# qianduoduolr/FGVC

Measured on AMD Instinct MI355X. Metric: frames/sec + ms/corr-volume, 480p 8-frame clip, 1/2/4/8 MI355X, higher is better.
Workload: dtype f16 + fp6 (e2m3) MFMA operands, f32 accumulate; top-k near-ties re-scored in f64 from f32 features

## Files before the change

### fgvc_amd/_lib.py

```python
from __future__ import annotations

import ctypes as C
import contextlib
import os

_HERE = os.path.dirname(os.path.abspath(__file__))
LIB_PATH = os.environ.get("FGVC_HIP_LIB") or os.path.join(_HERE, "lib", "libfgvc_hip.so")

FGVC_OK = 0
ERR_INVALID_ARG, ERR_UNSUPPORTED, ERR_LAUNCH = 1, 2, 3
NO_LIMIT = 0x3FFFFFFF
PAIR_MASKED = 1
WEIGHT_SOFTMAX, WEIGHT_COSINE, WEIGHT_RAW = 0, 1, 2

_p = C.c_void_p
_i = C.c_int
_f = C.c_float

SIGNATURES = {
    "fgvc_version": (C.c_char_p, []),
    "fgvc_last_error": (C.c_char_p, []),
    "fgvc_set_option": (_i, [C.c_char_p, _i]),
    "fgvc_r2max_for_radius": (_i, [_f]),
    "fgvc_normalize_chw_to_hwc_f32": (_i, [_p, _p, _i, _i, _i, _i, _i, _p]),
# ... 4 lines not shown
    "fgvc_split_f16f6p": (_i, [_p, _p, C.c_int64, _i, _p]),
    "fgvc_pair_topk_f16f6": (_i, [_p, _p, _p, _i, _i, _i, _i, _i, _i, _i, _i, _i, _i, _i, _p, _p, _p]),
    "fgvc_pair_topk_f16f6_runs": (_i, [_p, _p, _p, _i, _i, _i, _i, _i, _i, _i, _i, _i, _i, _i, _p, _i, _p, _p, _p]),
    "fgvc_split_f16f6x": (_i, [_p, _p, C.c_int64, _i, _p]),
    "fgvc_pair_topk_f16f6x": (_i, [_p, _p, _p, _i, _i, _i, _i, _i, _i, _i, _i, _i, _i, _i, _p, _p, _p]),
    "fgvc_pair_topk_f16f6x_runs": (_i, [_p, _p, _p, _i, _i, _i, _i, _i, _i, _i, _i, _i, _i, _i, _p, _i, _p, _p, _p]),
    "fgvc_merge_refine_workspace_bytes": (C.c_size_t, [_i, _i]),
    "fgvc_merge_refine_topk_f32": (_i, [_p, _p, _p, _p, _p, C.c_int64, _i, _p, C.c_int64, _i, _i, _i, _i, _i, _i, _i, _i, _i, _f, _i, _f, _i, _i, _i,
                                        _p, _p, _p, _p, _p]),
    "fgvc_pair_topk_f16x3_timed_out": (_i, []),
    "fgvc_pair_topk_f16x3_probe": (_i, [_p]),
    "fgvc_conv64_probe": (_i, [_p]),
    "fgvc_nchw_to_split_nhwc_f32": (_i, [_p, _p, _p, _i, _i, _i, _i, _i, _i, _p]),
    "fgvc_conv_split_f32": (_i, [_p, _p, _p, _p, _p, _p, _i, _i, _i, _i, _i, _i, _i, _i, _i, _p]),
    "fgvc_conv_split_fmt_f32": (_i, [_p, _p, _p, _p, _p, _p, _i, _i, _i, _i, _i, _i, _i, _i, _i, _i, _i, _i, _i, _p, _p]),
    "fgvc_conv_split_proj_fmt_f32": (_i, [_p, _p, _p, _p, _p, _p, _p, _p, _i, _i, _i, _i, _i, _i, _i, _i, _i, _i, _i, _i, _p, _p]),
    "fgvc_conv_split_bank_f16f6p_f32": (_i, [_p, _p, _p, _p, _p, _i, _i, _i, _i, _i, _i, _i, _i, _i, _i, _i, _p]),
    "fgvc_conv_split_bank_f16f6x_f32": (_i, [_p, _p, _p, _p, _p, _i, _i, _i, _i, _i, _i, _i, _i, _i, _i, _i, _p]),
    "fgvc_conv64_split_f32": (_i, [_p, _p, _p, _p, _p, _p, _i, _i, _i, _i, _i, _i, _p]),
    "fgvc_conv64_split_res_f32": (_i, [_p, _p, _p, _p, _p, _p, _p, _i, _i, _i, _i, _i, _i, _p]),
    "fgvc_conv64_split_fmt_f32": (_i, [_p, _p, _p, _p, _p, _p, _p, _i, _i, _i, _i, _i, _i, _i, _i, _i, _i, _p, _p]),
    "fgvc_conv_s2_split_f32": (_i, [_p, _p, _p, _p, _p, _i, _i, _i, _i, _i, _i, _i, _i, _i, _i, _i, _p]),
    "fgvc_conv_s2_split_fmt_f32": (_i, [_p, _p, _p, _p, _p, _i, _i, _i, _i, _i, _i, _i, _i, _i, _i, _i, _i, _i, _p, _p]),
    "fgvc_stem7_split_f32": (_i, [_p, _p, _p, _p, _p, _i, _i, _i, _i, _i, _i, _p]),
    "fgvc_stem7_split_fmt_f32": (_i, [_p, _p, _p, _p, _p, _i, _i, _i, _i, _i, _i, _i, _i, _p, _p]),
    "fgvc_nhwc_to_split_f32": (_i, [_p, _p, _i, _i, _i, _i, _i, _i, _i, _p]),
    "fgvc_normalize_nhwc_f32": (_i, [_p, _p, _i, _i, _i, _i, _i, _p]),
    "fgvc_normalize_split_nhwc_f32": (_i, [_p, _p, _p, _i, _i, _i, _i, _i, _p]),
    "fgvc_normalize_split_f16x2_nhwc_f32": (_i, [_p, _p, _p, _i, _i, _i, _i, _i, _p]),
    "fgvc_normalize_split_f16f6p_nhwc_f32": (_i, [_p, _p, _i, _i, _i, _i, _i, _p]),
    "fgvc_normalize_split_f16f6x_nhwc_f32": (_i, [_p, _p, _i, _i, _i, _i, _i, _p]),
    "fgvc_merge_topk_f32": (_i, [_p, _p, _p, _i, _i, _i, _i, _i, _f, _i, _p, _p, _p, _p]),
    "fgvc_propagate_topk_f32": (_i, [_p, _p, _i, _p, _p, _i, _i, _i, _i, _i, _i, _i, _p, _p]),
    "fgvc_corr_volume_f32": (_i, [_p, _p, _i, _i, _i, _f, _p, _p]),
    "fgvc_split_bf16": (_i, [_p, _p, C.c_int64, _i, _p]),
    "fgvc_corr_volume_bf16x3": (_i, [_p, _p, _i, _i, _i, _f, _p, _p]),
    "fgvc_corr_volume_bf16": (_i, [_p, _p, _i, _i, _i, _f, _p, _p]),
    "fgvc_split_f16f8": (_i, [_p, _p, C.c_int64, _i, _p]),
    "fgvc_corr_volume_f16f8": (_i, [_p, _p, _i, _i, _i, _f, _p, _p]),
    "fgvc_split_f16f6": (_i, [_p, _p, C.c_int64, _i, _p]),
    "fgvc_corr_volume_f16f6": (_i, [_p, _p, _i, _i, _i, _f, _p, _p]),
    "fgvc_debug_store_sweep_f32": (_i, [_p, C.c_int64, _i, _p]),
    "fgvc_dense_attend_splits": (_i, [_i, _i]),
    "fgvc_dense_attend_f32": (_i, [_p, _p, _i, _i, _i, _i, _i, _i, _i, _i, _i, _i, _i, _p, _i, _p]),
    "fgvc_dense_attend_finish_f32": (_i, [_p, _i, _i, _i, _i, _p, _p]),
    "fgvc_dense_kth_f32": (_i, [_p, _i, _i, _i, _p, _i, _p, _p]),
# ... 69 lines not shown
```

### fgvc_amd/csrc/capi.hip

```cpp
#include <stdarg.h>
#include <string.h>

#include "common.hpp"

namespace fgvc {

static thread_local char g_err[512] = "";

void set_error(const char* fmt, ...) {
  va_list ap;
  va_start(ap, fmt);
  vsnprintf(g_err, sizeof(g_err), fmt, ap);
  va_end(ap);
}

int pair_topk_launch(const float*, const float*, const int32_t*, int, int, int, int, int, int, int, int, int, int,
                     const uint8_t*, int32_t*, float*, hipStream_t);
int merge_topk_launch(const int32_t*, const float*, const int32_t*, int, int, int, int, int, float, int, int32_t*,
                      float*, float*, hipStream_t);
int normalize_launch(const float*, float*, int, int, int, int, int, hipStream_t);
int propagate_launch(const float*, const int32_t*, int, const int32_t*, const float*, int, int, int, int, int, int,
                     int, float*, hipStream_t);
int bn_act_launch(const float*, const float*, const float*, const float*, const float*, const float*, float, int, float*,
                  int, int, int, hipStream_t);
int gaussian_launch(const float*, int, int, int, int, float, float*, hipStream_t);
int softargmax_launch(const float*, int, int, int, int, int, int, const float*, float, double*, float*, hipStream_t);
int softargmax_bands();
int corr_volume_f32_launch(const float*, const float*, int, int, int, float, float*, hipStream_t);
int split_bf16_launch(const float*, uint16_t*, long long, int, hipStream_t);
int corr_volume_bf16_launch(const uint16_t*, const uint16_t*, int, int, int, float, float*, int, hipStream_t);
int local_merge_launch(const int32_t*, const float*, int, int, int, int, int, float, int32_t*, float*, float*,
                       hipStream_t);
int topk_coord_launch(const int32_t*, const float*, int, int, int, int, int, float*, hipStream_t);
int c2f_refine_launch(const int32_t*, const float*, const float*, const float*, int, int, int, int, int, int, int,
                      int, float, int, float*, int32_t*, float*, hipStream_t);

int conv_split_launch(const uint16_t*, const uint16_t*, const float*, const float*, uint16_t*, float*, int, int, int, int, int,
                      int, int, int, int, int, int, int, int, int*, hipStream_t, unsigned char* y_bank = nullptr, int bank_normalize = 1, const uint16_t* x2 = nullptr,
                      const uint16_t* w2 = nullptr, int Cin2 = 0, int bank_row_bytes = 1024);
int conv_s2_launch(const uint16_t*, const uint16_t*, const float*, uint16_t*, float*, int, int, int, int, int, int, int, int, int,
                   int, int, int, int, int*, hipStream_t);
int conv64_launch(const uint16_t*, const uint16_t*, const float*, const float*, const uint16_t*, uint16_t*, float*, int, int, int, int, int, int,
                  int, int, int, int, int*, hipStream_t);
int stem7_launch(const float*, const uint16_t*, const float*, uint16_t*, float*, int, int, int, int, int, int, int, int, int, int, int*,
                 hipStream_t);
int nchw_to_split_nhwc_launch(const float*, uint16_t*, float*, int, int, int, int, int, int, hipStream_t);
int normalize_nhwc_launch(const float*, float*, uint16_t*, int, int, int, int, int, int, hipStream_t);
int nhwc_to_split_launch(float*, uint16_t*, int, int, int, int, int, int, int, hipStream_t);

void set_conv_cot_cap(int);
void set_conv_narrow(int);
void set_conv64_variant(int);
int conv64_probe_read(long long*);
void set_conv_debug(int);
void set_corr6_skew(int);
void set_corr6_sdma(int);
void set_pair_debug(int);
void set_readout_prune(int);
void set_conv_s2_debug(int);
int split_f16x2_launch(const float*, uint16_t*, long long, int, hipStream_t);
int split_f16f6p_launch(const float*, unsigned char*, long long, int, hipStream_t);
int pair_topk_v7_launch(const uint16_t*, const uint16_t*, const int32_t*, int, int, int, int, int, int, int, int, int, const int32_t*, int,
                        int32_t*, float*, int, hipStream_t);
int pair_topk_v5_launch(const uint16_t*, const uint16_t*, const int32_t*, int, int, int, int, int, int, int, int, int, int, const int32_t*,
// ... 636 lines not shown

int fgvc_conv_s2_split_fmt_f32(const uint16_t* x, const uint16_t* w, const float* bias, uint16_t* y_split, float* y_f32, int N,
                               int H, int W, int Hp, int Wp, int Cin, int Cout, int KS, int Hop, int Wop, int relu, int out_fmt,
                               int out_scale_log2, int* overflow, void* stream) {
  FGVC_REQUIRE(x && w && bias && (y_split || y_f32), FGVC_ERR_INVALID_ARG, "fgvc_conv_s2_split_f32: null pointer");
  FGVC_REQUIRE(out_fmt >= 0 && out_fmt <= 3 && out_scale_log2 > -100 && out_scale_log2 < 100, FGVC_ERR_INVALID_ARG, "fgvc_conv_s2_split_fmt_f32: bad output format / scale");
  FGVC_REQUIRE(out_fmt == FGVC_ACT_BF16X2 || !y_split || overflow, FGVC_ERR_INVALID_ARG, "fgvc_conv_s2_split_fmt_f32: an f16-format output needs the overflow word");
  FGVC_REQUIRE(N >= 0 && H > 0 && W > 0, FGVC_ERR_INVALID_ARG, "fgvc_conv_s2_split_f32: bad shape");
  FGVC_REQUIRE(KS == 1 || KS == 3, FGVC_ERR_UNSUPPORTED, "fgvc_conv_s2_split_f32: kernel size %d (1 or 3, stride 2)", KS);
  FGVC_REQUIRE(Cin > 0 && Cin % 32 == 0 && Cout > 0 && Cout % 32 == 0, FGVC_ERR_UNSUPPORTED,
               "fgvc_conv_s2_split_f32: Cin=%d and Cout=%d must be multiples of 32", Cin, Cout);
  const int Ho = (H - 1) / 2 + 1, Wo = (W - 1) / 2 + 1;
  FGVC_REQUIRE(conv_pad_ok(H, W, Hp, Wp), FGVC_ERR_INVALID_ARG, "fgvc_conv_s2_split_f32: padded size %dx%d too small for %dx%d", Hp, Wp, H, W);
  FGVC_REQUIRE(!y_split || conv_pad_ok(Ho, Wo, Hop, Wop), FGVC_ERR_INVALID_ARG,
               "fgvc_conv_s2_split_f32: padded output size %dx%d too small for %dx%d", Hop, Wop, Ho, Wo);
  FGVC_REQUIRE(aligned16(x) && aligned16(w) && aligned16(bias) && aligned16(y_split) && aligned16(y_f32),
               FGVC_ERR_INVALID_ARG, "fgvc_conv_s2_split_f32: 16-byte alignment required");
  FGVC_REQUIRE((const void*)x != (const void*)y_split, FGVC_ERR_INVALID_ARG, "fgvc_conv_s2_split_f32: in-place not supported");
  if (N == 0) return FGVC_OK;
  return conv_s2_launch(x, w, bias, y_split, y_f32, N, Hp, Wp, Cin, Cout, KS, Ho, Wo, Hop, Wop, relu, out_fmt, out_scale_log2, overflow,
                        (hipStream_t)stream);
}

int fgvc_stem7_split_f32(const float* x, const uint16_t* w, const float* bias, uint16_t* y_split, float* y_f32, int N, int H,
                         int W, int Hop, int Wop, int relu, void* stream) {
  return fgvc_stem7_split_fmt_f32(x, w, bias, y_split, y_f32, N, H, W, Hop, Wop, relu, FGVC_ACT_BF16X2, 0, nullptr, stream);
}

int fgvc_stem7_split_fmt_f32(const float* x, const uint16_t* w, const float* bias, uint16_t* y_split, float* y_f32, int N, int H,
                             int W, int Hop, int Wop, int relu, int out_fmt, int out_scale_log2, int* overflow, void* stream) {
  FGVC_REQUIRE(x && w && bias && (y_split || y_f32), FGVC_ERR_INVALID_ARG, "fgvc_stem7_split_f32: null pointer");
  FGVC_REQUIRE(out_fmt == FGVC_ACT_BF16X2 || out_fmt == FGVC_ACT_F16F8, FGVC_ERR_UNSUPPORTED, "fgvc_stem7_split_fmt_f32: output format %d", out_fmt);
  FGVC_REQUIRE(out_fmt == FGVC_ACT_BF16X2 || !y_split || overflow, FGVC_ERR_INVALID_ARG,
               "fgvc_stem7_split_fmt_f32: an f16-format output needs the overflow word");
  FGVC_REQUIRE(out_scale_log2 > -100 && out_scale_log2 < 100, FGVC_ERR_INVALID_ARG, "fgvc_stem7_split_fmt_f32: scale exponent out of range");
  FGVC_REQUIRE(N >= 0 && H > 0 && W > 0, FGVC_ERR_INVALID_ARG, "fgvc_stem7_split_f32: bad shape");
  const int Ho = (H - 1) / 2 + 1, Wo = (W - 1) / 2 + 1;
  FGVC_REQUIRE(!y_split || conv_pad_ok(Ho, Wo, Hop, Wop), FGVC_ERR_INVALID_ARG,
               "fgvc_stem7_split_f32: padded output size %dx%d too small for %dx%d", Hop, Wop, Ho, Wo);
  FGVC_REQUIRE(aligned16(w) && aligned16(bias) && aligned16(y_split) && aligned16(y_f32) && ((uintptr_t)x & 3) == 0,
               FGVC_ERR_INVALID_ARG, "fgvc_stem7_split_f32: alignment (16 bytes; 4 for x)");
  if (N == 0) return FGVC_OK;
  return stem7_launch(x, w, bias, y_split, y_f32, N, H, W, Ho, Wo, Hop, Wop, relu, out_fmt, out_scale_log2, overflow, (hipStream_t)stream);
}

int fgvc_nhwc_to_split_f32(float* x, uint16_t* out, int N, int C, int H, int W, int Hp, int Wp, int relu, void* stream) {
// ... 72 lines not shown
```

### fgvc_amd/csrc/conv_s2.hip

```cpp
#include "common.hpp"

namespace fgvc {

struct ConvS2Params {
  const uint16_t* x;
  const uint16_t* w;
  const float* bias;
  uint16_t* y_split;
  float* y_f32;
  int N, Hp, Wp, Cin, Cout, Ho, Wo, Hop, Wop, relu;
  int n_ty, n_tx;
  int debug;
  float out_scale;
  int out_fmt;
  int* overflow;
};


__device__ __forceinline__ void s2_lds_dma_16(const void* src_lane, uint32_t lds_uniform) {
  asm volatile("s_mov_b32 m0, %1\n\ts_nop 0\n\tglobal_load_lds_dwordx4 %0, off" ::"v"(src_lane), "s"(lds_uniform) : "memory");
}
__device__ __forceinline__ uint32_t s2_lds_addr(const void* p) {
  return (uint32_t)(size_t)(const __attribute__((address_space(3))) unsigned char*)p;
}
__device__ __forceinline__ int s2_swz(int e, int s) { return e * 128 + ((s ^ ((e >> 1) & 7)) << 4); }

constexpr int S2_TR = 4;
constexpr int S2_NW = 2 * S2_TR;
constexpr int S2_CPG = 1;
constexpr int S2_RS = 144;

template <int KS>
__global__ __launch_bounds__(64 * S2_NW, 2) void conv_s2_kernel(ConvS2Params p) {
  constexpr int T = KS * KS;
  constexpr int NR = KS == 3 ? 2 * S2_TR + 1 : S2_TR;
  constexpr int NC = KS == 3 ? 65 : 32;
  constexpr int NE = NR * NC;
  constexpr int NG = (NE + 7) / 8;
// ... 180 lines not shown
    }
  }
}

static int g_conv_s2_debug = 0;
void set_conv_s2_debug(int v) { g_conv_s2_debug = v; }

int conv_s2_launch(const uint16_t* x, const uint16_t* w, const float* bias, uint16_t* y_split, float* y_f32, int N, int Hp,
                   int Wp, int Cin, int Cout, int KS, int Ho, int Wo, int Hop, int Wop, int relu, int out_fmt, int out_scale_log2,
                   int* overflow, hipStream_t s) {
  ConvS2Params p;
  p.out_fmt = out_fmt; p.out_scale = ldexpf(1.0f, out_scale_log2); p.overflow = overflow;
  p.x = x; p.w = w; p.bias = bias; p.y_split = y_split; p.y_f32 = y_f32;
  p.N = N; p.Hp = Hp; p.Wp = Wp; p.Cin = Cin; p.Cout = Cout; p.Ho = Ho; p.Wo = Wo; p.Hop = Hop; p.Wop = Wop; p.relu = relu;
  p.n_ty = cdiv(Ho, S2_TR); p.n_tx = cdiv(Wo, 32);
  p.debug = g_conv_s2_debug;
  dim3 grid(p.n_ty * p.n_tx * N, cdiv(Cout, 128));
  if (KS == 3) conv_s2_kernel<3><<<grid, 64 * S2_NW, 0, s>>>(p);
  else conv_s2_kernel<1><<<grid, 64 * S2_NW, 0, s>>>(p);
  FGVC_CHECK_LAUNCH("fgvc_conv_s2_split_f32");
  return FGVC_OK;
}

}
```

### fgvc_amd/mmpt_api/backbones.py

```python
from __future__ import annotations

import re
from typing import Sequence

import torch
import torch.nn as nn
import torch.nn.functional as F

from .registry import BACKBONES

_CAPTURING = [False]


class ConvBN(nn.Module):

    def __init__(self, cin, cout, k, stride=1, padding=0, dilation=1, relu=True):
        super().__init__()
        self.conv = nn.Conv2d(cin, cout, k, stride, padding, dilation, bias=False)
        self.bn = nn.BatchNorm2d(cout)
        self.relu = relu

    def forward(self, x, residual=None, relu=None):
        relu = self.relu if relu is None else relu
        y = self.conv(x)
# ... 80 lines not shown
            if self.torchvision_pretrain:
                load_torchvision_checkpoint(self, self.pretrained)
            elif isinstance(self.pretrained, str):
                load_checkpoint(self, self.pretrained)
            else:
                raise Exception("a state dict is only accepted as a torchvision checkpoint (resnet.py:590)")
            return
        for m in self.modules():
            if isinstance(m, nn.Conv2d):
                nn.init.kaiming_normal_(m.weight, mode="fan_out", nonlinearity="relu")
            elif isinstance(m, nn.BatchNorm2d):
                nn.init.constant_(m.weight, 1)
                nn.init.constant_(m.bias, 0)
        if self.zero_init_residual:
            for m in self.modules():
                if isinstance(m, BasicBlock):
                    nn.init.constant_(m.conv2.bn.weight, 0)
                elif isinstance(m, Bottleneck):
                    nn.init.constant_(m.conv3.bn.weight, 0)

    use_conv64 = True
    use_stem7 = True
    use_s2_conv = True
    conv64_f16f8 = True
    res_from_split = False
    use_split_conv = True
    arith = "f16f6"
    fold_projection = True
    layer1_whole_batch = True
    fuse_bank = True

    @staticmethod
    def supported_arith():
        return ("f16f6", "f16f8", "bf16x3", "f16x3")

    def set_arith(self, arith: str):
        if arith not in self.supported_arith():
            raise ValueError(f"arith={arith!r}: one of {self.supported_arith()}")
        if arith != self.arith:
            self.arith = arith
            self.reset_split_cache()

    def _generic_s1(self, cb) -> bool:
        c = cb.conv
        return c.stride == (1, 1) and not (self.use_conv64 and tuple(c.weight.shape) == (64, 64, 3, 3))

    def _is_conv64(self, cb) -> bool:
        c = cb.conv
        return bool(self.use_conv64 and c.stride == (1, 1) and tuple(c.weight.shape) == (64, 64, 3, 3))

    def _stem7_ok(self) -> bool:
        c1 = self.conv1.conv
        return bool(self.use_stem7 and c1.kernel_size == (7, 7) and c1.stride == (2, 2) and c1.padding == (3, 3) and c1.in_channels == 3
                    and c1.out_channels == 64 and c1.dilation == (1, 1) and self.conv1.relu)

    def _format_plan(self, last: int):
        from .. import ops
        fmt, bf = ops.ACT_FMT[self.arith], ops.ACT_BF16X2
        cache = self.__dict__.setdefault("_split_cache", {})
        key = ("fmt_plan", self.arith, last, self.use_conv64, self.use_s2_conv, self.use_stem7, self.conv64_f16f8)
        if key not in cache:
            blocks = [(s_i, b_i, blk) for s_i in range(last + 1) for b_i, blk in enumerate(getattr(self, self.res_layers[s_i]))]
            f64 = ops.ACT_F16F8 if (fmt in (ops.ACT_F16F8, ops.ACT_F16F6) and self.conv64_f16f8) else bf

            def reads(cb):
                if self._is_conv64(cb):
                    return f64
                return fmt if self._generic_s1(cb) else bf

            def can_write(cb, f):
                if f == bf:
                    return True
                if self._is_conv64(cb):
                    return f == ops.ACT_F16F8
                return self._generic_s1(cb) or (cb.conv.stride == (2, 2) and self.use_s2_conv)

            def wants(blk):
                f = reads(blk.conv1)
                return f if (blk.downsample is None or reads(blk.downsample) == f) else bf
            plan = {}
            f_in = wants(blocks[0][2]) if blocks else bf
            if f_in != bf and not (self._stem7_ok() and f_in == ops.ACT_F16F8):
                f_in = bf
# ... 241 lines not shown
            H, W = cur["H"], cur["W"]
            f_in, f_a, f_y = fmts[bi]
            s_in = cur.get("scale", 0)
            s_a = scales.get((si, bi, "a"), 0) if f_a != ACT_BF16X2 else 0
            s_y = scales.get((si, bi, "y"), 0) if f_y != ACT_BF16X2 else 0
            assert cur.get("fmt", ACT_BF16X2) == f_in, "split activation format mismatch between producer and consumer"

            def conv_s1(x_split, wb, in_fmt=ACT_BF16X2, in_scale=0, out_fmt=ACT_BF16X2, out_scale=0, **kw):
                if wb[3] == "conv64":
                    ops.conv64_split(x_split, wb[0], wb[1], H, W, in_fmt=in_fmt, in_scale_log2=in_scale + wb[2], out_fmt=out_fmt,
                                     out_scale_log2=out_scale, overflow=ovf, **kw)
                else:
                    ops.conv_split(x_split, wb[0], wb[1], H, W, in_fmt=in_fmt, in_scale_log2=in_scale + wb[2], out_fmt=out_fmt,
                                   out_scale_log2=out_scale, overflow=ovf, **kw)

            last_conv = bi == len(stage) - 1 and not cur["need_split"]
            proj = None
            x_in_split = cur["split"]
            if blk.conv1.conv.stride == (2, 2) and self.use_s2_conv:
                Hi, Wi = H, W
                H, W = (Hi - 1) // 2 + 1, (Wi - 1) // 2 + 1
                bufs = self._split_buffers((si, bi), N, Cout, H, W, dev, ("s_a", "s_y", "f_y", "f_idt"))
                buf = {k: v[lo:hi] for k, v in bufs.items()}
                ops.conv_s2_split(cur["split"], wt["ds"][0], wt["ds"][1], Hi, Wi, relu=False, out_f32=buf["f_idt"])
                idt = buf["f_idt"]
                ops.conv_s2_split(cur["split"], wt["c1"][0], wt["c1"][1], Hi, Wi, relu=True, out_split=buf["s_a"], out_fmt=f_a,
                                  out_scale_log2=s_a, overflow=ovf)
            elif blk.conv1.conv.stride != (1, 1):
                x_cl = cur["f32"].permute(0, 3, 1, 2)
                t1 = self._miopen_nhwc((si, bi, "c1"), blk.conv1, x_cl)
                idt = self._miopen_nhwc((si, bi, "ds"), blk.downsample, x_cl)
                _, H, W, _ = t1.shape
                bufs = self._split_buffers((si, bi), N, Cout, H, W, dev, ("s_a", "s_y", "f_y"))
                buf = {k: v[lo:hi] for k, v in bufs.items()}
                assert f_a == ACT_BF16X2
                ops.nhwc_to_split(t1, buf["s_a"], relu=True)
            else:
                bufs = self._split_buffers((si, bi), N, Cout, H, W, dev, ("s_a", "s_y", "f_y", "f_idt"))
                buf = {k: v[lo:hi] for k, v in bufs.items()}
                if blk.downsample is not None:
                    proj = self._projection_fold(blk, wt, si, bi, dev, f_in, f_a, s_in, s_a, Cout, last_conv and si == call["last"] and call.get("bank_of") is not None)
                if proj is not None:
                    idt = None
                elif blk.downsample is not None:
                    conv_s1(cur["split"], wt["ds"], f_in, s_in, relu=False, out_f32=buf["f_idt"])
                    idt = buf["f_idt"]
                elif self._identity_from_split(blk):
                    idt, idt_split = None, cur["split"]
                else:
                    idt = cur["f32"]
# ... 139 lines not shown
        for st in stages:
            x = st(x)
            outs.append(x)
        return outs[:-1], x, False, x.shape[-2], x.shape[-1]

    def forward(self, x, out_idx=None):
        want = tuple(out_idx) if out_idx is not None else self.out_indices
        last = max(want)
        earlier, y, nhwc, H, W = self._trunk(x, last, fresh=want)
        if nhwc:
            y = y.permute(0, 3, 1, 2)
        stage_out = earlier + [y]
        outs = [stage_out[i] for i in want]
        return outs[0] if len(outs) == 1 else tuple(outs)

    use_graph = "auto"
    graph_auto_max_px = 300_000

    def forward_hwc(self, x, normalize: bool = True, split_if=None, split_fmt: str = "bf16", out=None):
        want = self.use_graph is True or (self.use_graph == "auto" and x.dim() == 4 and x.shape[0] * x.shape[2] * x.shape[3] <= self.graph_auto_max_px)
        if not (want and x.is_cuda and not self.training and x.dtype == torch.float32) or torch.cuda.is_current_stream_capturing():
            return self.forward_hwc_eager(x, normalize, split_if, split_fmt, out)
        cache = self.__dict__.setdefault("_split_cache", {})
        sig = (self.arith, self.split_lanes, self.use_conv64, self.use_stem7, self.use_s2_conv, self.conv64_f16f8, self.res_from_split,
               self.use_split_conv, self.fuse_bank, self.fold_projection, self.layer1_whole_batch, tuple(self.out_indices))
        key = ("graph", tuple(x.shape), x.device, bool(normalize), split_fmt, split_if is not None, sig)
        ent = cache.get(key)
        if ent is None:
            cache[key] = "warm"
            return self.forward_hwc_eager(x, normalize, split_if, split_fmt, out)
        if ent == "warm":
            if self._scales(x.device) is None and self.arith != "bf16x3":
                return self.forward_hwc_eager(x, normalize, split_if, split_fmt, out)
            static_in = torch.empty_like(x)
            static_in.copy_(x)
            self.forward_hwc_eager(static_in, normalize, split_if, split_fmt, None)
            torch.cuda.synchronize(x.device)
            g = torch.cuda.CUDAGraph()
            _CAPTURING[0] = True
            try:
                with torch.cuda.graph(g):
                    o, H, W = self.forward_hwc_eager(static_in, normalize, split_if, split_fmt, None)
            finally:
                _CAPTURING[0] = False
            ent = cache[key] = (g, static_in, o, H, W)
        g, static_in, o, H, W = ent
        static_in.copy_(x)
# ... 97 lines not shown
```

### fgvc_amd/ops.py

```python
from __future__ import annotations

import ctypes as C
import functools
import math
from dataclasses import dataclass
from typing import Optional, Tuple

import torch

from . import _lib
from ._lib import NO_LIMIT, PAIR_MASKED, WEIGHT_COSINE, WEIGHT_RAW, WEIGHT_SOFTMAX


@dataclass(frozen=True)
class MaskSpec:
    r2max: int = NO_LIMIT
    ry: int = NO_LIMIT
    rx: int = NO_LIMIT

    @property
    def is_none(self) -> bool:
        return self.r2max >= NO_LIMIT and self.ry >= NO_LIMIT and self.rx >= NO_LIMIT

    @staticmethod
# ... 827 lines not shown


def conv_s2_split(x_split: torch.Tensor, w: torch.Tensor, bias: torch.Tensor, H: int, W: int, relu: bool,
                  out_split: Optional[torch.Tensor] = None, out_f32: Optional[torch.Tensor] = None, out_fmt: int = ACT_BF16X2,
                  out_scale_log2: int = 0, overflow: Optional[torch.Tensor] = None) -> None:
    x_split = _chk(x_split, torch.int16, "x_split")
    N, Hp, Wp, nch, _ = x_split.shape
    taps, nch_w, n_ct = w.shape[:3]
    Cout = n_ct * 32
    assert tuple(w.shape[3:]) == (4, 64, 8) and nch_w == nch and taps in (1, 9) and bias.shape == (Cout,)
    Ho, Wo = (H - 1) // 2 + 1, (W - 1) // 2 + 1
    Hop, Wop = conv_pad_dims(Ho, Wo)
    if out_split is not None:
        assert out_split.dtype == torch.int16 and tuple(out_split.shape) == (N, Hop, Wop, Cout // 32, 64) and out_split.is_contiguous()
    if out_f32 is not None:
        assert out_f32.dtype == torch.float32 and tuple(out_f32.shape) == (N, Ho, Wo, Cout) and out_f32.is_contiguous()
    if out_fmt != ACT_BF16X2 and out_split is not None:
        assert overflow is not None and overflow.dtype == torch.int32 and overflow.device == x_split.device
    _lib.call("fgvc_conv_s2_split_fmt_f32", _ptr(x_split), _ptr(w), _ptr(bias), _ptr(out_split), _ptr(out_f32), N, H, W, Hp, Wp,
              nch * 32, Cout, 3 if taps == 9 else 1, Hop, Wop, int(relu), int(out_fmt), int(out_scale_log2), _ptr(overflow),
              _stream(x_split))


def stem7_split(x: torch.Tensor, w: torch.Tensor, bias: torch.Tensor, relu: bool = True,
                out_split: Optional[torch.Tensor] = None, out_f32: Optional[torch.Tensor] = None, out_fmt: int = ACT_BF16X2,
                out_scale_log2: int = 0, overflow: Optional[torch.Tensor] = None) -> None:
    x = _chk(x, torch.float32, "x")
    N, C, H, W = x.shape
    assert C == 3 and x.is_contiguous() and tuple(w.shape) == (7, 2, 2, 2, 64, 8) and bias.shape == (64,)
    Ho, Wo = (H - 1) // 2 + 1, (W - 1) // 2 + 1
    Hop, Wop = conv_pad_dims(Ho, Wo)
    if out_split is not None:
        assert out_split.dtype == torch.int16 and tuple(out_split.shape) == (N, Hop, Wop, 2, 64) and out_split.is_contiguous()
    if out_f32 is not None:
        assert out_f32.dtype == torch.float32 and tuple(out_f32.shape) == (N, Ho, Wo, 64) and out_f32.is_contiguous()
    _lib.call("fgvc_stem7_split_fmt_f32", _ptr(x), _ptr(w), _ptr(bias), _ptr(out_split), _ptr(out_f32), N, H, W, Hop, Wop,
              int(relu), int(out_fmt), int(out_scale_log2), _ptr(overflow), _stream(x))


def normalize_nhwc(x: torch.Tensor, normalize: bool = True, split=False, out: Optional[torch.Tensor] = None) -> torch.Tensor:
    fmt = "bf16" if split is True else split
    assert fmt in (False, "bf16", "f16", "f16f6", "f16f6x")
    x = _chk(x, torch.float32, "x")
    N, H, W, C = x.shape
    shape, dt = ((N, H * W, 4 if fmt == "f16f6x" else 2, C), torch.int16) if split else ((N, H * W, C), torch.float32)
    if out is None:
# ... 120 lines not shown
```

### include/fgvc_hip.h

```cpp
#ifndef FGVC_HIP_H
#define FGVC_HIP_H

#include <stddef.h>
#include <stdint.h>

#ifdef __cplusplus
extern "C" {
#endif

#define FGVC_OK 0
#define FGVC_ERR_INVALID_ARG 1
#define FGVC_ERR_UNSUPPORTED 2
#define FGVC_ERR_LAUNCH 3

#define FGVC_NO_LIMIT 0x3fffffff

#define FGVC_PAIR_MASKED 1

#define FGVC_WEIGHT_SOFTMAX 0
#define FGVC_WEIGHT_COSINE 1
#define FGVC_WEIGHT_RAW 2

const char* fgvc_version(void);
const char* fgvc_last_error(void);
// ... 121 lines not shown
                                 int Cin2, int relu, int in_fmt, int in_scale_log2, int out_fmt, int out_scale_log2, int* overflow,
                                 void* stream);
int fgvc_conv_split_bank_f16f6p_f32(const uint16_t* x, const uint16_t* w, const float* bias, const float* residual, void* bank,
                                    int N, int H, int W, int Hp, int Wp, int Cin, int KS, int relu, int in_fmt, int in_scale_log2,
                                    int normalize, void* stream);
int fgvc_conv_split_bank_f16f6x_f32(const uint16_t* x, const uint16_t* w, const float* bias, const float* residual, void* bank,
                                    int N, int H, int W, int Hp, int Wp, int Cin, int KS, int relu, int in_fmt, int in_scale_log2,
                                    int normalize, void* stream);
int fgvc_conv64_split_f32(const uint16_t* x, const uint16_t* w, const float* bias, const float* residual, uint16_t* y_split,
                          float* y_f32, int N, int H, int W, int Hp, int Wp, int relu, void* stream);
int fgvc_conv64_split_fmt_f32(const uint16_t* x, const uint16_t* w, const float* bias, const float* residual,
                              const uint16_t* residual_split, uint16_t* y_split, float* y_f32, int N, int H, int W, int Hp, int Wp,
                              int relu, int in_fmt, int in_scale_log2, int out_fmt, int out_scale_log2, int* overflow, void* stream);
int fgvc_conv64_probe(int64_t* out32);
int fgvc_conv64_split_res_f32(const uint16_t* x, const uint16_t* w, const float* bias, const float* residual,
                              const uint16_t* residual_split, uint16_t* y_split, float* y_f32, int N, int H, int W, int Hp, int Wp,
                              int relu, void* stream);
int fgvc_conv_s2_split_f32(const uint16_t* x, const uint16_t* w, const float* bias, uint16_t* y_split, float* y_f32, int N,
                           int H, int W, int Hp, int Wp, int Cin, int Cout, int KS, int Hop, int Wop, int relu,
                           void* stream);
int fgvc_conv_s2_split_fmt_f32(const uint16_t* x, const uint16_t* w, const float* bias, uint16_t* y_split, float* y_f32, int N,
                               int H, int W, int Hp, int Wp, int Cin, int Cout, int KS, int Hop, int Wop, int relu, int out_fmt,
                               int out_scale_log2, int* overflow, void* stream);
int fgvc_stem7_split_f32(const float* x, const uint16_t* w, const float* bias, uint16_t* y_split, float* y_f32, int N, int H,
                         int W, int Hop, int Wop, int relu, void* stream);
int fgvc_stem7_split_fmt_f32(const float* x, const uint16_t* w, const float* bias, uint16_t* y_split, float* y_f32, int N, int H,
                             int W, int Hop, int Wop, int relu, int out_fmt, int out_scale_log2, int* overflow, void* stream);
int fgvc_normalize_nhwc_f32(const float* in, float* out, int N, int C, int H, int W, int normalize, void* stream);
int fgvc_normalize_split_nhwc_f32(const float* in, float* out_f32, uint16_t* out_split, int N, int C, int H, int W,
                                  int normalize, void* stream);
int fgvc_normalize_split_f16x2_nhwc_f32(const float* in, float* out_f32, uint16_t* out_split, int N, int C, int H, int W,
                                        int normalize, void* stream);
int fgvc_normalize_split_f16f6p_nhwc_f32(const float* in, uint8_t* rows, int N, int C, int H, int W, int normalize, void* stream);
int fgvc_normalize_split_f16f6x_nhwc_f32(const float* in, uint8_t* rows, int N, int C, int H, int W, int normalize, void* stream);

int fgvc_gaussian_labels_f32(const float* points, int P, int Hf, int Wf, int stride, float sigma,
                             float* out, void* stream);

size_t fgvc_softargmax_workspace_bytes(int n_frames, int P);
int fgvc_softargmax_top5_f32(const float* labels, int n_frames, int Hf, int Wf, int P, int h, int w,
                             const float* gauss_points, float sigma, double* coords, void* workspace,
                             void* stream);

int fgvc_seg_max_label_u8(const uint8_t* map, int hp, int wp, int Hf, int Wf, int32_t* out, void* stream);
int fgvc_seg_onehot_labels_u8(const uint8_t* map, int hp, int wp, int Hf, int Wf, int C, float* out, void* stream);

// ... 11 lines not shown
```

Baseline: 1999.

## Fuse stride-2 conv1 and 1x1 downsample projection into one persistent kernel

Adds a persistent stride-2 block kernel that computes the 3x3 conv1 (ReLU, split output) and the 1x1 downsample projection (f32 output) from the same LDS-staged input patch. The projection reuses the center-tap (t==4) activations, so the input is read once instead of twice. Tiles are spread across one workgroup per CU, with double-buffered global_load_lds DMA prefetching the next tile's chunks. The block is enabled by default in the backbone; it raises register pressure from the second accumulator set and adds an extra epilogue pass through LDS.

New measurement: 1994, median of 2. About the same (-0.2%).

```diff
diff --git a/fgvc_amd/_lib.py b/fgvc_amd/_lib.py
--- a/fgvc_amd/_lib.py
+++ b/fgvc_amd/_lib.py
@@ -50,6 +50,7 @@
     "fgvc_conv64_split_fmt_f32": (_i, [_p, _p, _p, _p, _p, _p, _p, _i, _i, _i, _i, _i, _i, _i, _i, _i, _i, _p, _p]),
     "fgvc_conv_s2_split_f32": (_i, [_p, _p, _p, _p, _p, _i, _i, _i, _i, _i, _i, _i, _i, _i, _i, _i, _p]),
     "fgvc_conv_s2_split_fmt_f32": (_i, [_p, _p, _p, _p, _p, _i, _i, _i, _i, _i, _i, _i, _i, _i, _i, _i, _i, _i, _p, _p]),
+    "fgvc_conv_s2_block_fmt_f32": (_i, [_p, _p, _p, _p, _p, _p, _p, _i, _i, _i, _i, _i, _i, _i, _i, _i, _i, _i, _p, _p]),
     "fgvc_stem7_split_f32": (_i, [_p, _p, _p, _p, _p, _i, _i, _i, _i, _i, _i, _p]),
     "fgvc_stem7_split_fmt_f32": (_i, [_p, _p, _p, _p, _p, _i, _i, _i, _i, _i, _i, _i, _i, _p, _p]),
     "fgvc_nhwc_to_split_f32": (_i, [_p, _p, _i, _i, _i, _i, _i, _i, _i, _p]),
diff --git a/fgvc_amd/csrc/capi.hip b/fgvc_amd/csrc/capi.hip
--- a/fgvc_amd/csrc/capi.hip
+++ b/fgvc_amd/csrc/capi.hip
@@ -40,6 +40,8 @@
                       const uint16_t* w2 = nullptr, int Cin2 = 0, int bank_row_bytes = 1024);
 int conv_s2_launch(const uint16_t*, const uint16_t*, const float*, uint16_t*, float*, int, int, int, int, int, int, int, int, int,
                    int, int, int, int, int*, hipStream_t);
+int conv_s2_block_launch(const uint16_t*, const uint16_t*, const float*, const uint16_t*, const float*, uint16_t*, float*, int, int, int,
+                         int, int, int, int, int, int, int, int, int*, hipStream_t);
 int conv64_launch(const uint16_t*, const uint16_t*, const float*, const float*, const uint16_t*, uint16_t*, float*, int, int, int, int, int, int,
                   int, int, int, int, int*, hipStream_t);
 int stem7_launch(const float*, const uint16_t*, const float*, uint16_t*, float*, int, int, int, int, int, int, int, int, int, int, int*,
@@ -722,6 +724,28 @@
                         (hipStream_t)stream);
 }
 
+int fgvc_conv_s2_block_fmt_f32(const uint16_t* x, const uint16_t* w, const float* bias, const uint16_t* w_p, const float* bias_p,
+                               uint16_t* y_split, float* y_proj, int N, int H, int W, int Hp, int Wp, int Cin, int Cout, int Hop, int Wop,
+                               int out_fmt, int out_scale_log2, int* overflow, void* stream) {
+  FGVC_REQUIRE(x && w && bias && w_p && bias_p && y_split && y_proj, FGVC_ERR_INVALID_ARG, "fgvc_conv_s2_block_fmt_f32: null pointer");
+  FGVC_REQUIRE(out_fmt >= 0 && out_fmt <= 3 && out_scale_log2 > -100 && out_scale_log2 < 100, FGVC_ERR_INVALID_ARG, "fgvc_conv_s2_block_fmt_f32: bad output format / scale");
+  FGVC_REQUIRE(out_fmt == FGVC_ACT_BF16X2 || overflow, FGVC_ERR_INVALID_ARG, "fgvc_conv_s2_block_fmt_f32: an f16-format output needs the overflow word");
+  FGVC_REQUIRE(N >= 0 && H > 0 && W > 0, FGVC_ERR_INVALID_ARG, "fgvc_conv_s2_block_fmt_f32: bad shape");
+  FGVC_REQUIRE(Cin > 0 && Cin % 32 == 0 && Cout > 0 && Cout % 32 == 0, FGVC_ERR_UNSUPPORTED,
+               "fgvc_conv_s2_block_fmt_f32: Cin=%d and Cout=%d must be multiples of 32", Cin, Cout);
+  const int Ho = (H - 1) / 2 + 1, Wo = (W - 1) / 2 + 1;
+  FGVC_REQUIRE(conv_pad_ok(H, W, Hp, Wp), FGVC_ERR_INVALID_ARG, "fgvc_conv_s2_block_fmt_f32: padded size %dx%d too small for %dx%d", Hp, Wp, H, W);
+  FGVC_REQUIRE(conv_pad_ok(Ho, Wo, Hop, Wop), FGVC_ERR_INVALID_ARG,
+               "fgvc_conv_s2_block_fmt_f32: padded output size %dx%d too small for %dx%d", Hop, Wop, Ho, Wo);
+  FGVC_REQUIRE(aligned16(x) && aligned16(w) && aligned16(bias) && aligned16(w_p) && aligned16(bias_p) && aligned16(y_split) && aligned16(y_proj),
+               FGVC_ERR_INVALID_ARG, "fgvc_conv_s2_block_fmt_f32: 16-byte alignment required");
+  FGVC_REQUIRE((const void*)x != (const void*)y_split && (const void*)x != (const void*)y_proj, FGVC_ERR_INVALID_ARG,
+               "fgvc_conv_s2_block_fmt_f32: in-place not supported");
+  if (N == 0) return FGVC_OK;
+  return conv_s2_block_launch(x, w, bias, w_p, bias_p, y_split, y_proj, N, Hp, Wp, Cin, Cout, Ho, Wo, Hop, Wop, out_fmt, out_scale_log2,
+                              overflow, (hipStream_t)stream);
+}
+
 int fgvc_stem7_split_f32(const float* x, const uint16_t* w, const float* bias, uint16_t* y_split, float* y_f32, int N, int H,
                          int W, int Hop, int Wop, int relu, void* stream) {
   return fgvc_stem7_split_fmt_f32(x, w, bias, y_split, y_f32, N, H, W, Hop, Wop, relu, FGVC_ACT_BF16X2, 0, nullptr, stream);
diff --git a/fgvc_amd/csrc/conv_s2.hip b/fgvc_amd/csrc/conv_s2.hip
--- a/fgvc_amd/csrc/conv_s2.hip
+++ b/fgvc_amd/csrc/conv_s2.hip
@@ -14,6 +14,10 @@
   float out_scale;
   int out_fmt;
   int* overflow;
+  const uint16_t* w_p;
+  const float* bias_p;
+  float* y_proj;
+  int tiles_per_wg;
 };
 
 
@@ -240,4 +244,246 @@
   return FGVC_OK;
 }
 
-}
+constexpr int S2P_NR = 2 * S2_TR + 1, S2P_NC = 65, S2P_NE = S2P_NR * S2P_NC;
+constexpr int S2P_NG = (S2P_NE + 7) / 8;
+constexpr int S2P_CHUNKB = S2P_NG * 1024;
+constexpr int S2P_PW = (S2P_NG + S2_NW - 1) / S2_NW;
+static_assert(2 * S2P_CHUNKB <= 160 * 1024 && S2_NW * 32 * S2_RS <= S2P_CHUNKB, "LDS: two patch buffers, the epilogue tiles in one");
+static_assert(S2P_PW <= 9 + 1, "pieces: one per tap, two at the last");
+
+__device__ __forceinline__ void s2p_lds_dma_16(const void* src_lane, uint32_t lds_uniform) {
+  asm volatile("s_mov_b32 m0, %1\n\ts_nop 0\n\tglobal_load_lds_dwordx4 %0, off" ::"v"(src_lane), "s"(lds_uniform) : "memory", "m0");
+}
+
+__global__ __launch_bounds__(64 * S2_NW, 2) void conv_s2p_kernel(ConvS2Params p) {
+  constexpr int NC = S2P_NC, NE = S2P_NE, NG = S2P_NG, CHUNKB = S2P_CHUNKB;
+  __shared__ __attribute__((aligned(16))) unsigned char smem[2 * CHUNKB];
+  auto wave_sync = [&]() { asm volatile("s_waitcnt lgkmcnt(0)" ::: "memory"); };
+
+  const int tid = threadIdx.x, lane = tid & 63;
+  const int wave = __builtin_amdgcn_readfirstlane(tid >> 6);
+  const int ct = wave & 3, half = wave >> 2;
+  const int n = lane & 31, h = lane >> 5;
+  const int d_row = lane >> 3, d_slot = lane & 7;
+  const int nchunk = p.Cin / 32, n_ct = p.Cout / 32;
+  const size_t pix_bytes_in = (size_t)nchunk * 128;
+  const int tiles_img = p.n_ty * p.n_tx;
+  const int ntiles = tiles_img * p.N * cdiv(p.Cout, 128);
+  const int t_begin = blockIdx.x * p.tiles_per_wg, t_end = imin(ntiles, t_begin + p.tiles_per_wg);
+  if (t_begin >= t_end) return;
+
+  auto dma = [&](int tile, int chunk, int g, unsigned char* buf) {
+    int r = tile % (tiles_img * p.N);
+    const int nimg = r / tiles_img;
+    r -= nimg * tiles_img;
+    const int ty = r / p.n_tx, tx = r - ty * p.n_tx;
+    const int e = imin(g * 8 + d_row, NE - 1);
+    const int j = e / NC, m = e - j * NC;
+    int prow = 2 * ty * S2_TR + j, pcol = 2 * tx * 32 + (m < 33 ? 2 * m : 2 * (m - 33) + 1);
+    if (prow >= p.Hp || pcol >= p.Wp) prow = pcol = 0;
+    const int sl = d_slot ^ ((e >> 1) & 7);
+    const unsigned char* src = reinterpret_cast<const unsigned char*>(p.x) +
+                               (((size_t)nimg * p.Hp + prow) * p.Wp + pcol) * pix_bytes_in + (size_t)chunk * 128 + sl * 16;
+    s2p_lds_dma_16(src, s2_lds_addr(buf + g * 1024));
+  };
+  if (!(p.debug & 1)) {
+#pragma unroll
+    for (int q = 0; q < S2P_PW; ++q)
+      if (wave + S2_NW * q < NG) dma(t_begin, 0, wave + S2_NW * q, smem);
+  }
+
+  int k = 0;
+  for (int tile = t_begin; tile < t_end; ++tile) {
+    int r = tile % (tiles_img * p.N);
+    const int cb = tile / (tiles_img * p.N);
+    const int nimg = r / tiles_img;
+    r -= nimg * tiles_img;
+    const int ty = r / p.n_tx, tx = r - ty * p.n_tx;
+    const int y0 = ty * S2_TR, x0 = tx * 32;
+    const int co_w = cb * 128 + ct * 32;
+    const bool active = co_w < p.Cout;
+    const uint16_t* wlane = p.w + (size_t)(active ? (co_w >> 5) : 0) * 2048 + lane * 8;
+    const uint16_t* wlane_p = p.w_p + (size_t)(active ? (co_w >> 5) : 0) * 2048 + lane * 8;
+    f32x4 bias_v[4];
+#pragma unroll
+    for (int g = 0; g < 4; ++g) bias_v[g] = *reinterpret_cast<const f32x4*>(p.bias + (active ? co_w : 0) + 8 * g + 4 * h);
+
+    f32x16 acc[2], accp[2];
+#pragma unroll
+    for (int b = 0; b < 2; ++b)
+#pragma unroll
+      for (int q = 0; q < 16; ++q) acc[b][q] = accp[b][q] = 0.f;
+
+    for (int c = 0; c < nchunk; ++c, ++k) {
+      const unsigned char* patch = smem + (k & 1) * CHUNKB;
+      unsigned char* nbuf = smem + ((k + 1) & 1) * CHUNKB;
+      const bool last_c = c + 1 == nchunk;
+      const int ntile = last_c ? tile + 1 : tile, nchunk_i = last_c ? 0 : c + 1;
+      const bool has_next = ntile < t_end && !(p.debug & 1);
+      asm volatile("s_waitcnt vmcnt(0)" ::: "memory");
+      __syncthreads();
+
+      bf16x8 a_cur[4], a_nxt[4], a_p[4];
+      auto load_a = [&](bf16x8* a, int t) {
+        const uint16_t* wp = wlane + ((size_t)t * nchunk + c) * n_ct * 2048;
+#pragma unroll
+        for (int q = 0; q < 4; ++q) a[q] = *reinterpret_cast<const bf16x8*>((p.debug & 8) ? wlane + q * 512 : wp + q * 512);
+      };
+#pragma unroll
+      for (int q = 0; q < 4; ++q)
+        a_p[q] = *reinterpret_cast<const bf16x8*>((p.debug & 8) ? wlane_p + q * 512 : wlane_p + (size_t)c * n_ct * 2048 + q * 512);
+      load_a(a_cur, 0);
+      for (int t = 0; t < 9; ++t) {
+        if (t + 1 < 9) load_a(a_nxt, t + 1);
+        if (has_next) {
+          if (wave + S2_NW * t < NG) dma(ntile, nchunk_i, wave + S2_NW * t, nbuf);
+          if (t == 8 && S2P_PW > 9 && wave + S2_NW * 9 < NG) dma(ntile, nchunk_i, wave + S2_NW * 9, nbuf);
+        }
+        __builtin_amdgcn_sched_barrier(0);
+        const int dy = t / 3, dx = t - 3 * (t / 3);
+        const int mbase = dx == 0 ? 0 : dx == 1 ? 33 : 1;
+#pragma unroll
+        for (int b = 0; b < 2; ++b) {
+          const int e = (2 * (half * 2 + b) + dy) * NC + mbase + n;
+          bf16x8 xh[2], xl[2];
+#pragma unroll
+          for (int s = 0; s < 2; ++s) {
+            xh[s] = *reinterpret_cast<const bf16x8*>(patch + s2_swz(e, 2 * s + h));
+            xl[s] = *reinterpret_cast<const bf16x8*>(patch + s2_swz(e, 4 + 2 * s + h));
+          }
+          if (p.debug & 2) {
+            acc[b][0] += (float)(xh[0][0] + xl[0][0] + xh[1][0] + xl[1][0] + a_cur[0][0] + a_cur[1][0] + a_cur[2][0] + a_cur[3][0]);
+            continue;
+          }
+#pragma unroll
+          for (int s = 0; s < 2; ++s) {
+            acc[b] = __builtin_amdgcn_mfma_f32_32x32x16_bf16(a_cur[s], xh[s], acc[b], 0, 0, 0);
+            acc[b] = __builtin_amdgcn_mfma_f32_32x32x16_bf16(a_cur[2 + s], xh[s], acc[b], 0, 0, 0);
+            acc[b] = __builtin_amdgcn_mfma_f32_32x32x16_bf16(a_cur[s], xl[s], acc[b], 0, 0, 0);
+          }
+          if (t == 4) {
+#pragma unroll
+            for (int s = 0; s < 2; ++s) {
+              accp[b] = __builtin_amdgcn_mfma_f32_32x32x16_bf16(a_p[s], xh[s], accp[b], 0, 0, 0);
+              accp[b] = __builtin_amdgcn_mfma_f32_32x32x16_bf16(a_p[2 + s], xh[s], accp[b], 0, 0, 0);
+              accp[b] = __builtin_amdgcn_mfma_f32_32x32x16_bf16(a_p[s], xl[s], accp[b], 0, 0, 0);
+            }
+          }
+        }
+#pragma unroll
+        for (int q = 0; q < 4; ++q) a_cur[q] = a_nxt[q];
+      }
+    }
+    __syncthreads();
+    if (!active || (p.debug & 4)) continue;
+
+    unsigned char* tile_lds = smem + ((k - 1) & 1) * CHUNKB + wave * (32 * S2_RS);
+    const int mv_row = lane >> 3, mv_col = (lane & 7) * 16;
+    f32x4 biasp_v[4];
+#pragma unroll
+    for (int g = 0; g < 4; ++g) biasp_v[g] = *reinterpret_cast<const f32x4*>(p.bias_p + co_w + 8 * g + 4 * h);
+#pragma unroll
+    for (int b = 0; b < 2; ++b) {
+      const int y = y0 + half * 2 + b;
+      if (y >= p.Ho) continue;
+#pragma unroll
+      for (int g = 0; g < 4; ++g) {
+        const f32x4 bv = biasp_v[g];
+        const f32x4 v = {accp[b][4 * g + 0] + bv.x, accp[b][4 * g + 1] + bv.y, accp[b][4 * g + 2] + bv.z, accp[b][4 * g + 3] + bv.w};
+        *reinterpret_cast<f32x4*>(tile_lds + n * S2_RS + (8 * g + 4 * h) * 4) = v;
+      }
+      wave_sync();
+      {
+        unsigned char* dst = reinterpret_cast<unsigned char*>(p.y_proj + (((size_t)nimg * p.Ho + y) * p.Wo + x0) * p.Cout + co_w);
+#pragma unroll
+        for (int i = 0; i < 4; ++i) {
+          const int row = i * 8 + mv_row;
+          if (x0 + row < p.Wo)
+            *reinterpret_cast<uint4*>(dst + (size_t)row * p.Cout * 4 + mv_col) = *reinterpret_cast<const uint4*>(tile_lds + row * S2_RS + mv_col);
+        }
+      }
+      wave_sync();
+      f32x4 v[4];
+#pragma unroll
+      for (int g = 0; g < 4; ++g) {
+        const f32x4 bv = bias_v[g];
+        v[g] = {acc[b][4 * g + 0] + bv.x, acc[b][4 * g + 1] + bv.y, acc[b][4 * g + 2] + bv.z, acc[b][4 * g + 3] + bv.w};
+        v[g].x = fmaxf(v[g].x, 0.f); v[g].y = fmaxf(v[g].y, 0.f); v[g].z = fmaxf(v[g].z, 0.f); v[g].w = fmaxf(v[g].w, 0.f);
+      }
+      unsigned char* o = tile_lds + n * S2_RS;
+      if (p.out_fmt == 0) {
+#pragma unroll
+        for (int g = 0; g < 4; ++g) {
+          ushort4 hv, lv;
+          split_bf16_4(v[g], hv, lv);
+          *reinterpret_cast<ushort4*>(o + (8 * g + 4 * h) * 2) = hv;
+          *reinterpret_cast<ushort4*>(o + 64 + (8 * g + 4 * h) * 2) = lv;
+        }
+      } else if (p.out_fmt == 3) {
+        bool ovf = false;
+        uint2 hw[4];
+        fgvc_i32x4 main6, tail6;
+        split_f16f6_chunk(v, p.out_scale, h, hw, main6, tail6, ovf);
+#pragma unroll
+        for (int g = 0; g < 4; ++g) *reinterpret_cast<uint2*>(o + (8 * g + 4 * h) * 2) = hw[g];
+        *reinterpret_cast<fgvc_i32x4*>(o + 80 - 16 * h) = main6;
+        *reinterpret_cast<fgvc_i32x4*>(o + 112 - 16 * h) = tail6;
+        if (__builtin_amdgcn_ballot_w64(ovf && x0 + n < p.Wo) != 0ull && lane == 0) atomicOr(p.overflow, 1);
+      } else {
+        bool ovf = false;
+#pragma unroll
+        for (int g = 0; g < 4; ++g) {
+          uint2 hw, lw;
+          uint32_t l8, h8;
+          split_f16_4(v[g], p.out_scale, hw, l8, h8, lw, ovf);
+          *reinterpret_cast<uint2*>(o + (8 * g + 4 * h) * 2) = hw;
+          if (p.out_fmt == 1) {
+            *reinterpret_cast<uint32_t*>(o + 64 + 8 * g + 4 * h) = l8;
+            *reinterpret_cast<uint32_t*>(o + 96 + 8 * g + 4 * h) = h8;
+          } else {
+            *reinterpret_cast<uint2*>(o + 64 + (8 * g + 4 * h) * 2) = lw;
+          }
+        }
+        if (__builtin_amdgcn_ballot_w64(ovf && x0 + n < p.Wo) != 0ull && lane == 0) atomicOr(p.overflow, 1);
+      }
+      wave_sync();
+      const size_t pix0 = ((size_t)nimg * p.Hop + (y + 1)) * p.Wop + (x0 + 1);
+      unsigned char* dst = reinterpret_cast<unsigned char*>(p.y_split) + (pix0 * (p.Cout / 32) + (co_w >> 5)) * 128;
+#pragma unroll
+      for (int i = 0; i < 4; ++i) {
+        const int row = i * 8 + mv_row;
+        if (x0 + row < p.Wo)
+          *reinterpret_cast<uint4*>(dst + (size_t)row * p.Cout * 4 + mv_col) = *reinterpret_cast<const uint4*>(tile_lds + row * S2_RS + mv_col);
+      }
+      wave_sync();
+    }
+  }
+}
+
+int conv_s2_block_launch(const uint16_t* x, const uint16_t* w, const float* bias, const uint16_t* w_p, const float* bias_p,
+                         uint16_t* y_split, float* y_proj, int N, int Hp, int Wp, int Cin, int Cout, int Ho, int Wo, int Hop, int Wop,
+                         int out_fmt, int out_scale_log2, int* overflow, hipStream_t s) {
+  static int n_cu[64] = {0};
+  int dev = 0;
+  FGVC_REQUIRE(hipGetDevice(&dev) == hipSuccess && dev >= 0 && dev < 64, FGVC_ERR_LAUNCH, "fgvc_conv_s2_block_fmt_f32: no current device");
+  if (n_cu[dev] == 0) {
+    int v = 0;
+    FGVC_REQUIRE(hipDeviceGetAttribute(&v, hipDeviceAttributeMultiprocessorCount, dev) == hipSuccess && v > 0, FGVC_ERR_LAUNCH,
+                 "fgvc_conv_s2_block_fmt_f32: CU count");
+    n_cu[dev] = v;
+  }
+  ConvS2Params p;
+  p.out_fmt = out_fmt; p.out_scale = ldexpf(1.0f, out_scale_log2); p.overflow = overflow;
+  p.x = x; p.w = w; p.bias = bias; p.y_split = y_split; p.y_f32 = nullptr;
+  p.w_p = w_p; p.bias_p = bias_p; p.y_proj = y_proj;
+  p.N = N; p.Hp = Hp; p.Wp = Wp; p.Cin = Cin; p.Cout = Cout; p.Ho = Ho; p.Wo = Wo; p.Hop = Hop; p.Wop = Wop; p.relu = 1;
+  p.n_ty = cdiv(Ho, S2_TR); p.n_tx = cdiv(Wo, 32);
+  p.debug = g_conv_s2_debug;
+  const int ntiles = p.n_ty * p.n_tx * N * cdiv(Cout, 128);
+  p.tiles_per_wg = cdiv(ntiles, n_cu[dev]);
+  conv_s2p_kernel<<<cdiv(ntiles, p.tiles_per_wg), 64 * S2_NW, 0, s>>>(p);
+  FGVC_CHECK_LAUNCH("fgvc_conv_s2_block_fmt_f32");
+  return FGVC_OK;
+}
+
+}
diff --git a/fgvc_amd/mmpt_api/backbones.py b/fgvc_amd/mmpt_api/backbones.py
--- a/fgvc_amd/mmpt_api/backbones.py
+++ b/fgvc_amd/mmpt_api/backbones.py
@@ -126,6 +126,7 @@
     use_conv64 = True
     use_stem7 = True
     use_s2_conv = True
+    use_s2_block = True
     conv64_f16f8 = True
     res_from_split = False
     use_split_conv = True
@@ -162,7 +163,7 @@
         from .. import ops
         fmt, bf = ops.ACT_FMT[self.arith], ops.ACT_BF16X2
         cache = self.__dict__.setdefault("_split_cache", {})
-        key = ("fmt_plan", self.arith, last, self.use_conv64, self.use_s2_conv, self.use_stem7, self.conv64_f16f8)
+        key = ("fmt_plan", self.arith, last, self.use_conv64, self.use_s2_conv, self.use_s2_block, self.use_stem7, self.conv64_f16f8)
         if key not in cache:
             blocks = [(s_i, b_i, blk) for s_i in range(last + 1) for b_i, blk in enumerate(getattr(self, self.res_layers[s_i]))]
             f64 = ops.ACT_F16F8 if (fmt in (ops.ACT_F16F8, ops.ACT_F16F6) and self.conv64_f16f8) else bf
@@ -450,10 +451,14 @@
                 H, W = (Hi - 1) // 2 + 1, (Wi - 1) // 2 + 1
                 bufs = self._split_buffers((si, bi), N, Cout, H, W, dev, ("s_a", "s_y", "f_y", "f_idt"))
                 buf = {k: v[lo:hi] for k, v in bufs.items()}
-                ops.conv_s2_split(cur["split"], wt["ds"][0], wt["ds"][1], Hi, Wi, relu=False, out_f32=buf["f_idt"])
+                if self.use_s2_block:
+                    ops.conv_s2_block(cur["split"], wt["c1"][0], wt["c1"][1], wt["ds"][0], wt["ds"][1], Hi, Wi, out_split=buf["s_a"],
+                                      out_proj=buf["f_idt"], out_fmt=f_a, out_scale_log2=s_a, overflow=ovf)
+                else:
+                    ops.conv_s2_split(cur["split"], wt["ds"][0], wt["ds"][1], Hi, Wi, relu=False, out_f32=buf["f_idt"])
+                    ops.conv_s2_split(cur["split"], wt["c1"][0], wt["c1"][1], Hi, Wi, relu=True, out_split=buf["s_a"], out_fmt=f_a,
+                                      out_scale_log2=s_a, overflow=ovf)
                 idt = buf["f_idt"]
-                ops.conv_s2_split(cur["split"], wt["c1"][0], wt["c1"][1], Hi, Wi, relu=True, out_split=buf["s_a"], out_fmt=f_a,
-                                  out_scale_log2=s_a, overflow=ovf)
             elif blk.conv1.conv.stride != (1, 1):
                 x_cl = cur["f32"].permute(0, 3, 1, 2)
                 t1 = self._miopen_nhwc((si, bi, "c1"), blk.conv1, x_cl)
@@ -639,7 +644,7 @@
         if not (want and x.is_cuda and not self.training and x.dtype == torch.float32) or torch.cuda.is_current_stream_capturing():
             return self.forward_hwc_eager(x, normalize, split_if, split_fmt, out)
         cache = self.__dict__.setdefault("_split_cache", {})
-        sig = (self.arith, self.split_lanes, self.use_conv64, self.use_stem7, self.use_s2_conv, self.conv64_f16f8, self.res_from_split,
+        sig = (self.arith, self.split_lanes, self.use_conv64, self.use_stem7, self.use_s2_conv, self.use_s2_block, self.conv64_f16f8, self.res_from_split,
                self.use_split_conv, self.fuse_bank, self.fold_projection, self.layer1_whole_batch, tuple(self.out_indices))
         key = ("graph", tuple(x.shape), x.device, bool(normalize), split_fmt, split_if is not None, sig)
         ent = cache.get(key)
diff --git a/fgvc_amd/ops.py b/fgvc_amd/ops.py
--- a/fgvc_amd/ops.py
+++ b/fgvc_amd/ops.py
@@ -873,6 +873,25 @@
               _stream(x_split))
 
 
+def conv_s2_block(x_split: torch.Tensor, w: torch.Tensor, bias: torch.Tensor, w_proj: torch.Tensor, bias_proj: torch.Tensor, H: int, W: int,
+                  out_split: torch.Tensor, out_proj: torch.Tensor, out_fmt: int = ACT_BF16X2, out_scale_log2: int = 0,
+                  overflow: Optional[torch.Tensor] = None) -> None:
+    x_split = _chk(x_split, torch.int16, "x_split")
+    N, Hp, Wp, nch, _ = x_split.shape
+    Cout = w.shape[2] * 32
+    assert tuple(w.shape) == (9, nch, Cout // 32, 4, 64, 8) and tuple(w_proj.shape) == (1, nch, Cout // 32, 4, 64, 8)
+    assert bias.shape == (Cout,) and bias_proj.shape == (Cout,)
+    Ho, Wo = (H - 1) // 2 + 1, (W - 1) // 2 + 1
+    Hop, Wop = conv_pad_dims(Ho, Wo)
+    assert out_split.dtype == torch.int16 and tuple(out_split.shape) == (N, Hop, Wop, Cout // 32, 64) and out_split.is_contiguous()
+    assert out_proj.dtype == torch.float32 and tuple(out_proj.shape) == (N, Ho, Wo, Cout) and out_proj.is_contiguous()
+    if out_fmt != ACT_BF16X2:
+        assert overflow is not None and overflow.dtype == torch.int32 and overflow.device == x_split.device
+    _lib.call("fgvc_conv_s2_block_fmt_f32", _ptr(x_split), _ptr(w), _ptr(bias), _ptr(w_proj), _ptr(bias_proj), _ptr(out_split),
+              _ptr(out_proj), N, H, W, Hp, Wp, nch * 32, Cout, Hop, Wop, int(out_fmt), int(out_scale_log2), _ptr(overflow),
+              _stream(x_split))
+
+
 def stem7_split(x: torch.Tensor, w: torch.Tensor, bias: torch.Tensor, relu: bool = True,
                 out_split: Optional[torch.Tensor] = None, out_f32: Optional[torch.Tensor] = None, out_fmt: int = ACT_BF16X2,
                 out_scale_log2: int = 0, overflow: Optional[torch.Tensor] = None) -> None:
diff --git a/include/fgvc_hip.h b/include/fgvc_hip.h
--- a/include/fgvc_hip.h
+++ b/include/fgvc_hip.h
@@ -167,6 +167,9 @@
 int fgvc_conv_s2_split_fmt_f32(const uint16_t* x, const uint16_t* w, const float* bias, uint16_t* y_split, float* y_f32, int N,
                                int H, int W, int Hp, int Wp, int Cin, int Cout, int KS, int Hop, int Wop, int relu, int out_fmt,
                                int out_scale_log2, int* overflow, void* stream);
+int fgvc_conv_s2_block_fmt_f32(const uint16_t* x, const uint16_t* w, const float* bias, const uint16_t* w_p, const float* bias_p,
+                               uint16_t* y_split, float* y_proj, int N, int H, int W, int Hp, int Wp, int Cin, int Cout, int Hop, int Wop,
+                               int out_fmt, int out_scale_log2, int* overflow, void* stream);
 int fgvc_stem7_split_f32(const float* x, const uint16_t* w, const float* bias, uint16_t* y_split, float* y_f32, int N, int H,
                          int W, int Hop, int Wop, int relu, void* stream);
 int fgvc_stem7_split_fmt_f32(const float* x, const uint16_t* w, const float* bias, uint16_t* y_split, float* y_f32, int N, int H,
```
